# multimodallearning/DG-TTA

Measured on AMD Instinct MI355X. Metric: TTA-epochs/sec per GPU on 128^3 patch; Dice delta vs reference, higher is better.
Workload: dtype fp16

## Files before the change

dg_tta_amd/_lib.py:

```python
import ctypes as C
import os
from pathlib import Path

LIB_PATH = Path(__file__).resolve().parent / "libdgtta_hip.so"

_c_float_p = C.POINTER(C.c_float)
P, I, I64, F, SZ = C.c_void_p, C.c_int, C.c_int64, C.c_float, C.c_size_t

SIGNATURES = {
    "dgtta_version": (I, []),
    "dgtta_last_error": (C.c_char_p, []),
    "dgtta_reload_env": (I, []),
    "dgtta_mind3d_ws_bytes": (SZ, [I, I, I, I]),
    "dgtta_mind3d_fwd": (I, [P, P, F, I, C.POINTER(F), I, P, I, I, I, P, SZ, I, I, I, I, P]),
    "dgtta_gin_ws_bytes": (SZ, [I, I, I, I]),
    "dgtta_gin_chain_fwd": (I, [P, P, C.POINTER(I), C.POINTER(P), C.POINTER(P), P, P, SZ, I, I, I, I, P]),
    "dgtta_affine_warp3d_fwd": (I, [P, P, P, I, I, I, I, I, I, I, I, I, I, I, I, I, I, P, P]),
    "dgtta_affine_warp3d_bwd": (I, [P, P, P, I, I, I, I, I, I, I, I, I, I, I, I, I, P]),
    "dgtta_softdice_ws_bytes": (SZ, [I, I, I64]),
    "dgtta_softdice_fwd": (I, [P, P, P, P, P, SZ, I, I, I64, I, I, I, P]),
    "dgtta_softdice_bwd": (I, [P, P, P, P, P, F, P, I, I, I64, I, I, P]),
    "dgtta_softdice_bwd_t": (I, [P, P, P, P, P, F, P, I, I, I64, I, I, I, P]),
    "dgtta_softdice_probs_fwd": (I, [P, P, P, P, SZ, I, I, I64, I64, I64, I64, P]),
    "dgtta_softdice_probs_bwd": (I, [P, P, P, P, P, P, I, I, I64, I64, I64, I64, P]),
# ... 6 lines not shown
    "dgtta_conv3d_packed_bytes": (SZ, [I, I, I]),
    "dgtta_conv3d_pack_weights": (I, [P, P, I, I, I, I, I, P]),
    "dgtta_conv3d_stats_bytes": (SZ, [I, I, I, I, I]),
    "dgtta_conv3d_k3_fwd": (I, [P, I, P, P, P, I, P, I, I, I, I, I, I, I, I, I, I, I, P]),
    "dgtta_conv3d_k3_dgrad": (I, [P, I, P, P, I, I, I, I, I, I, I, I, I, I, I, I, I, P]),
    "dgtta_conv3d_wgrad_ws_bytes": (SZ, [I, I, I, I, I, I]),
    "dgtta_conv3d_wgrad_split_ws_bytes": (SZ, [I, I, I, I, I, I, I]),
    "dgtta_conv3d_k3_wgrad": (I, [P, I, P, I, P, P, P, SZ, I, I, I, I, I, I, I, I, I, I, P]),
    "dgtta_conv3d_k3_blocked_supported": (I, [I, I, I, I, I, I, I]),
    "dgtta_conv3d_k3_fwd_blocked": (I, [P, I64, P, P, P, I, P, I, I, I, I, I, I, I, I, I, P]),
    "dgtta_conv3d_k3_wgrad_blocked": (I, [P, I64, P, I, P, P, P, SZ, I, I, I, I, I, I, I, I, P]),
    "dgtta_instnorm_ws_bytes": (SZ, [I, I, I64]),
    "dgtta_instnorm_lrelu_fwd": (I, [P, I, P, P, P, P, P, I, P, SZ, I, I, I64, F, F, I, P]),
    "dgtta_instnorm_lrelu_bwd": (I, [P, I, P, I, P, P, P, P, I, P, P, P, SZ, I, I, I64, F, I, I, P]),
    "dgtta_conv3d_k3_dgrad_gstats": (I, [P, I, P, P, I, I, I, I, I, I, I, I, I, P, I, P, P, P, F, P, SZ, C.POINTER(I), I, I, P]),
    "dgtta_instnorm_lrelu_bwd_gstats": (I, [P, I, P, I, P, P, P, P, I, P, P, P, P, SZ, I, I, I64, F, I, I, P]),
    "dgtta_convT3d_fwd_ws_bytes": (SZ, [I, I, I]),
    "dgtta_convT3d_k2s2_fwd": (I, [P, I, P, P, P, I, P, SZ, I, I, I, I, I, I, I, I, P]),
    "dgtta_convT3d_bwd_ws_bytes": (SZ, [I, I, I, I, I, I]),
    "dgtta_convT3d_bwd_split_ws_bytes": (SZ, [I, I, I, I, I, I]),
    "dgtta_convT3d_k2s2_bwd": (I, [P, I, P, I, P, P, I, P, P, P, SZ, I, I, I, I, I, I, I, I, I, P]),
    "dgtta_seghead_fwd": (I, [P, I, P, P, P, I, P, I, I, I, I, I64, I, P]),
    "dgtta_seghead_bwd_ws_bytes": (SZ, [I, I, I, I64]),
    "dgtta_seghead_bwd": (I, [P, I, P, I, P, P, I, P, I, P, P, P, SZ, I, I, I64, I, I, P]),
    "dgtta_seghead_warp_supported": (I, [P, I, I, I, I, I, I, I]),
    "dgtta_seghead_warp_bwd_ws_bytes": (SZ, [I, I, I, I, I, I]),
    "dgtta_seghead_warp_fwd": (I, [P, P, P, P, I, P, P, I, I, I, I, I, I, I, P]),
    "dgtta_seghead_warp_bwd": (I, [P, P, P, P, P, P, I, P, P, P, P, SZ, I, I, I, I, I, I, I, I, P]),
    "dgtta_seghead_warp_bwd_g16": (I, [P, P, P, P, P, P, I, P, P, P, P, SZ, I, I, I, I, I, I, I, I, P]),
    "dgtta_ncdhw_to_ndhwc": (I, [P, P, I, I, I64, I, I, P]),
# ... 69 lines not shown
```

dg_tta_amd/csrc/common.h:

```cpp
#pragma once
#include <hip/hip_runtime.h>
#include <hip/hip_bf16.h>
#include <hip/hip_fp16.h>
#include <stdint.h>
#include <stdio.h>
#include <stdarg.h>

#include "../../include/dgtta.h"

#define WAVE 64

#include <atomic>

void dgtta_set_error(const char *fmt, ...);

struct DgttaSwitches {
  int conv_rows, conv_s2, dgrad_s2_allcls, wgrad_tr, wgrad_tr8, wgrad_s2_onepass, convt_wgrad_onepass;
  int convt_gemm, rows_order, in_nt, wgrad_upw, wgrad_xcd, in_gstats, softdice16, conv_ring, wgrad_ring, ha_mfma, wgrad_f32_split, feature_head_mfma, headwarp_mfma, wgrad_flat, wgrad_reduce_taps;
  int rows_abl, rows_var, ring_nt, ring_abl, wgrad_ring_lab, ha_abl, warp_abl, convt_gemm_abl;
  int ncu;
};
const DgttaSwitches &dgtta_switches();
#ifdef DGTTA_DIAG
#define DG_LAB(field) (dgtta_switches().field)
// ... 11 lines not shown
  (void)hipGetDevice(&dev);
  const unsigned long long bit = 1ull << (dev & 63);
  if (o.mask.load(std::memory_order_acquire) & bit) return hipSuccess;
  const hipError_t e = hipFuncSetAttribute(fn, hipFuncAttributeMaxDynamicSharedMemorySize, bytes);
  if (e == hipSuccess) o.mask.fetch_or(bit, std::memory_order_release);
  return e;
}

struct RowsGstCtx {
  const void *y;
  long long ldy;
  const float *mr, *gamma, *beta;
  float slope;
  double *out;
  int produced;
};

#define DG_REQUIRE(cond, code, ...)      \
  do {                                   \
    if (!(cond)) {                       \
      dgtta_set_error(__VA_ARGS__);      \
      return (code);                     \
    }                                    \
  } while (0)

#define DG_CHECK_LAUNCH(name)                                                     \
  do {                                                                            \
    hipError_t e__ = hipGetLastError();                                           \
    if (e__ != hipSuccess) {                                                      \
      dgtta_set_error("%s: launch failed: %s", name, hipGetErrorString(e__));     \
// ... 94 lines not shown
```

dg_tta_amd/csrc/conv_mfma.hip:

```cpp
#include "conv_common.h"
#include <stdlib.h>
#include <type_traits>

int conv3_rows_launch(const void *x, const View &xv, const void *w, const Taps &taps, const float *bias, void *y, const View &yv,
                      int B, int Cin, int Cout, int CinP, int CoutP, double *stats, int ntaps_src, int is_f16, hipStream_t st,
                      RowsGstCtx *gst);

int conv3_ring_launch(const void *x, const View &xv, const void *w, const Taps &taps, const float *bias, void *y, const View &yv,
                      int B, int Cin, int Cout, int CinP, int CoutP, double *stats, int64_t stats_cap_slots, int ntaps_src,
                      int is_f16, hipStream_t st, RowsGstCtx *gst, long long xkh = 0, bool dry = false);
int64_t conv3_mfma_max_tiles(int Do, int Ho, int Wo);

namespace {

template <typename T, int MBW, int MBH, int MBD, int S, int NB, int KSPC, int ABL = 0, int NW = 4, bool AC = false>
__global__ __launch_bounds__(NW * 64) void conv3_mfma_kernel(const T *__restrict__ x, View xv, const T *__restrict__ w,
                                                         ConvClasses cs, const float *__restrict__ bias,
                                                         T *__restrict__ y, View yv, int Cin, int Cout, int CinP,
                                                         int CoutP, int tilesW, int tilesH, int tilesD,
                                                         double *__restrict__ stats, int ntaps_src) {
  const int cls = blockIdx.z;
  x += cs.xoff[cls];
  if (!AC) y += cs.yoff[cls];
  const Taps &taps = cs.taps[cls];
  const int accumulate = cs.acc[cls];
  const int Di = xv.D, Hi = xv.H, Wi = xv.W, Do = yv.D, Ho = yv.H, Wo = yv.W;
  typedef ConvCfg<T, MBW, MBH, MBD, S, NB, KSPC> Cfg;
  typedef typename Cfg::G G;
  constexpr int EPV = Cfg::EPV, NG = Cfg::NG, CK = Cfg::CK, NC = Cfg::NC, NV = G::NV, MPW = G::MB / NW, NT = NW * 64;
  extern __shared__ __attribute__((aligned(16))) unsigned char smem[];
  uint4 *sA = reinterpret_cast<uint4 *>(smem);
  uint4 *sB = reinterpret_cast<uint4 *>(smem + Cfg::A_BYTES);

  const int tid = threadIdx.x, lane = tid & 63, wave = tid >> 6;
  const int r = lane & 31, h = lane >> 5;
// ... 158 lines not shown
            else mfma_step<T>(af, bf[j], acc[i][j]);
          }
        }
      }
    }
  }

  float st1[NB], st2[NB];
#pragma unroll
  for (int j = 0; j < NB; ++j) st1[j] = st2[j] = 0.f;
  if (AC) {
    const bool vec = Cout % 8 == 0 && (reinterpret_cast<uintptr_t>(y) & 15) == 0 && yv.sw % 8 == 0 && yv.sh % 8 == 0 &&
                     yv.sd % 8 == 0 && yv.sb % 8 == 0;
    __syncthreads();
    float *slab = reinterpret_cast<float *>(smem) + wave * (32 * 36);
#pragma unroll
    for (int i = 0; i < MPW; ++i) {
      const int mb = wave * MPW + i;
      const int mbd = mb / MBH, mbh = mb % MBH;
      const int co = n0 + r;
      uint4 olds[8][2];
      if constexpr (sizeof(T) == 2) {
        if (vec && accumulate) {
#pragma unroll
          for (int c8 = 0; c8 < 8; ++c8)
#pragma unroll
            for (int t = 0; t < 2; ++t) {
              const int m = t * 16 + (lane >> 2), cq = (lane & 3) * 8;
              const int od = od0 + mbd, oh = oh0 + mbh * G::RPM + m / MBW, ow = ow0 + m % MBW;
              olds[c8][t] = make_uint4(0u, 0u, 0u, 0u);
              if (n0 + cq < Cout && od < Do && oh < Ho && ow < Wo)
                olds[c8][t] = *reinterpret_cast<const uint4 *>(y + cs.yoff[c8] + b * yv.sb + od * yv.sd + oh * yv.sh + ow * yv.sw + n0 + cq);
            }
        }
      }
#pragma unroll
      for (int c8 = 0; c8 < 8; ++c8) {
        if (!vec) {
#pragma unroll
          for (int q = 0; q < 16; ++q) {
            const int m = (q & 3) + 8 * (q >> 2) + 4 * h;
            const int od = od0 + mbd, oh = oh0 + mbh * G::RPM + m / MBW, ow = ow0 + m % MBW;
            if (co < Cout && od < Do && oh < Ho && ow < Wo) {
              T *o = y + cs.yoff[c8] + b * yv.sb + od * yv.sd + oh * yv.sh + ow * yv.sw + co;
              float v = acc[i][c8][q];
              if (accumulate) v += ld_f<T>(o);
              st_f<T>(o, v);
            }
          }
          continue;
        }
#pragma unroll
// ... 14 lines not shown
                const unsigned wv[4] = {old.x, old.y, old.z, old.w};
#pragma unroll
                for (int e = 0; e < 4; ++e) {
                  float lo, hi;
                  unpack2_16<T>(wv[e], lo, hi);
                  v[2 * e] += lo;
                  v[2 * e + 1] += hi;
                }
              }
              uint4 pk;
              pk.x = pack2_16<T>(v[0], v[1]);
              pk.y = pack2_16<T>(v[2], v[3]);
              pk.z = pack2_16<T>(v[4], v[5]);
              pk.w = pack2_16<T>(v[6], v[7]);
              *o4 = pk;
            } else {
              float4 *o4 = reinterpret_cast<float4 *>(o);
              if (accumulate) {
                const float4 a0 = o4[0], a1 = o4[1];
                v[0] += a0.x; v[1] += a0.y; v[2] += a0.z; v[3] += a0.w;
                v[4] += a1.x; v[5] += a1.y; v[6] += a1.z; v[7] += a1.w;
              }
              o4[0] = make_float4(v[0], v[1], v[2], v[3]);
              o4[1] = make_float4(v[4], v[5], v[6], v[7]);
            }
          }
        }
      }
    }
    return;
  }
#pragma unroll
  for (int i = 0; i < MPW; ++i) {
    const int mb = wave * MPW + i;
    const int mbd = mb / MBH, mbh = mb % MBH;
#pragma unroll
    for (int j = 0; j < NB; ++j) {
      const int co = n0 + j * 32 + r;
      const float bv = (bias && co < Cout) ? bias[co] : 0.f;
#pragma unroll
      for (int q = 0; q < 16; ++q) {
        const int m = (q & 3) + 8 * (q >> 2) + 4 * h;
        const int od = od0 + mbd, oh = oh0 + mbh * G::RPM + m / MBW, ow = ow0 + m % MBW;
// ... 30 lines not shown
#pragma unroll
      for (int wv = 0; wv < NW; ++wv) {
        s += (double)red[(wv * NC + tid) * 2 + 0];
        ss += (double)red[(wv * NC + tid) * 2 + 1];
      }
      double *p = stats + 32 + (((int64_t)b * tiles_per_b + (tlin % tiles_per_b)) * Cout + n0 + tid) * 2;
      p[0] = s;
      p[1] = ss;
    }
    if (blockIdx.x == 0 && blockIdx.y == 0 && tid == 0) reinterpret_cast<long long *>(stats)[0] = tiles_per_b;
  }
}

template <typename T, int MBW, int MBH, int MBD>
int launch_conv_allcls(const void *x, const View &xv, const void *w, const ConvClasses &cs, void *y, const View &yv, int B,
                       int Cin, int Cout, int CinP, int CoutP, hipStream_t st) {
  typedef ConvCfg<T, MBW, MBH, MBD, 1, 1, 1> Cfg;
  typedef typename Cfg::G G;
  auto kern = conv3_mfma_kernel<T, MBW, MBH, MBD, 1, 1, 1, 0, 8, true>;
  static DynLdsOnce lds_once;
  DG_REQUIRE(ensure_dyn_lds(lds_once, reinterpret_cast<const void *>(kern), (int)Cfg::LDS_BYTES) == hipSuccess,
             DGTTA_ERR_LAUNCH, "conv3_mfma: cannot raise the dynamic LDS limit to %zu", (size_t)Cfg::LDS_BYTES);
  const int tW = cdiv(yv.W, G::TW), tH = cdiv(yv.H, G::TH), tD = cdiv(yv.D, G::TD);
  const int64_t tiles = (int64_t)tW * tH * tD * B;
  DG_REQUIRE(tiles < (1ll << 31), DGTTA_ERR_UNSUPPORTED, "conv3_mfma: too many tiles");
  dim3 grid((unsigned)tiles, (unsigned)cdiv(CoutP, Cfg::NC), 1u);
  hipLaunchKernelGGL(kern, grid, dim3(8 * 64), Cfg::LDS_BYTES, st, (const T *)x, xv, (const T *)w, cs, (const float *)nullptr,
                     (T *)y, yv, Cin, Cout, CinP, CoutP, tW, tH, tD, (double *)nullptr, 27);
  DG_CHECK_LAUNCH("conv3_mfma_kernel<all classes>");
  return DGTTA_OK;
}

template <typename T, int MBW, int MBH, int MBD, int S, int NB, int KSPC, int NW = 4>
int launch_conv(const void *x, const View &xv, const void *w, const ConvClasses &cs, const float *bias, void *y,
                const View &yv, int B, int Cin, int Cout, int CinP, int CoutP, double *stats, int ntaps_src,
                hipStream_t st) {
  typedef ConvCfg<T, MBW, MBH, MBD, S, NB, KSPC> Cfg;
  typedef typename Cfg::G G;
  auto kern = conv3_mfma_kernel<T, MBW, MBH, MBD, S, NB, KSPC, 0, NW>;
  static DynLdsOnce lds_once;
  DG_REQUIRE(ensure_dyn_lds(lds_once, reinterpret_cast<const void *>(kern), (int)Cfg::LDS_BYTES) == hipSuccess,
             DGTTA_ERR_LAUNCH, "conv3_mfma: cannot raise the dynamic LDS limit to %zu", (size_t)Cfg::LDS_BYTES);
  const int tW = cdiv(yv.W, G::TW), tH = cdiv(yv.H, G::TH), tD = cdiv(yv.D, G::TD);
  const int64_t tiles = (int64_t)tW * tH * tD * B;
  DG_REQUIRE(tiles < (1ll << 31), DGTTA_ERR_UNSUPPORTED, "conv3_mfma: too many tiles");
  dim3 grid((unsigned)tiles, (unsigned)cdiv(CoutP, Cfg::NC), (unsigned)cs.n);
  hipLaunchKernelGGL(kern, grid, dim3(NW * 64), Cfg::LDS_BYTES, st, (const T *)x, xv, (const T *)w, cs, bias, (T *)y, yv,
                     Cin, Cout, CinP, CoutP, tW, tH, tD, stats, ntaps_src);
  DG_CHECK_LAUNCH("conv3_mfma_kernel");
  return DGTTA_OK;
}

template <typename T>
int dispatch_conv_classes(const void *x, const View &xv, const void *w, const ConvClasses &cs, const float *bias, void *y,
                          const View &yv, int B, int Cin, int Cout, int CinP, int CoutP, int stride, hipStream_t st,
                          double *stats = nullptr, int ntaps_src = 27, RowsGstCtx *gst = nullptr, long long xkh = 0, bool dry = false) {
#define ARGS x, xv, w, cs, bias, y, yv, B, Cin, Cout, CinP, CoutP, stats, ntaps_src, st
  const long long vox = (long long)yv.D * yv.H * yv.W * B;
  if ((xkh || dry) && stride != 1) return DGTTA_ERR_UNSUPPORTED;
  if (stride == 0) {
    if (yv.W >= 32) return launch_conv<T, 32, 4, 4, 0, 1, 1, 8>(ARGS);
    if (yv.W >= 16) return launch_conv<T, 16, 4, 4, 0, 1, 1, 8>(ARGS);
    if (vox <= 4096) return launch_conv<T, 8, 2, 2, 0, 1, 1>(ARGS);
// ... 89 lines not shown
    if (i < nf) {
      int ci = (int)(i % CinP), co = (int)((i / CinP) % CoutN), tap = (int)(i / ((int64_t)CinP * CoutN));
      st_f<T>(imgF + conv_weight_image_index(co, ci, tap, CinP, 27, EPV),
              (ci < Cin && co < Cout) ? w[((int64_t)co * Cin + ci) * 27 + tap] : 0.f);
    }
    if (i < nb) {
      int co = (int)(i % CoutP), ci = (int)((i / CoutP) % CinN), tap = (int)(i / ((int64_t)CoutP * CinN));
      st_f<T>(imgB + conv_weight_image_index(ci, co, tap, CoutP, 27, EPV),
              (ci < Cin && co < Cout) ? w[((int64_t)co * Cin + ci) * 27 + tap] : 0.f);
    }
  }
}

}

int64_t conv3_mfma_max_tiles(int Do, int Ho, int Wo) {
  const int shapes[6][3] = {{4, 4, 32}, {4, 8, 16}, {2, 8, 8}, {8, 8, 8}, {4, 4, 16}, {4, 8, 8}};
  int64_t best = 0;
  for (auto &t : shapes) {
    int64_t n = (int64_t)cdiv(Do, t[0]) * cdiv(Ho, t[1]) * cdiv(Wo, t[2]);
    best = n > best ? n : best;
  }
  return best;
}

int conv3_s2_regs(const void *x, const View &xv, const void *wimg, const float *bias, void *y, const View &yv, int B, int Cin,
                  int Cout, int CinP, int CoutP, double *stats, int64_t cap_slots, int dtype, hipStream_t st);

int conv3_fwd_mfma(const void *x, int ldx, const void *w_kmajor, int mirror, const float *bias, void *y, int ldy, int B,
                   int Cin, int Cout, int CinP, int CoutP, int Di, int Hi, int Wi, int stride, int dtype,
// ... 12 lines not shown
    return dispatch_conv<float>(x, xv, w_kmajor, taps, bias, y, yv, B, Cin, Cout, CinP, CoutP, stride, 0, st, stats, 27, gst);
  }
  if (dtype == DGTTA_BF16) {
    if (!operand_ok<bf16_t>(x, xkh ? 2 * ldx : ldx, Cin, CinP)) return DGTTA_ERR_UNSUPPORTED;
    return dispatch_conv<bf16_t>(x, xv, w_kmajor, taps, bias, y, yv, B, Cin, Cout, CinP, CoutP, stride, 0, st, stats, 27, gst, xkh, dry);
  }
  if (dtype == DGTTA_F16) {
    if (!operand_ok<f16_t>(x, xkh ? 2 * ldx : ldx, Cin, CinP)) return DGTTA_ERR_UNSUPPORTED;
    return dispatch_conv<f16_t>(x, xv, w_kmajor, taps, bias, y, yv, B, Cin, Cout, CinP, CoutP, stride, 0, st, stats, 27, gst, xkh, dry);
  }
  return DGTTA_ERR_UNSUPPORTED;
}

template <typename T>
static int dgrad_s2(const void *dy, int lddy, const void *w_kmajor, void *dx, int lddx, int B, int Cin, int Cout, int CinP,
                    int CoutP, int Di, int Hi, int Wi, int accumulate, hipStream_t st) {
  if (!operand_ok<T>(dy, lddy, Cout, CoutP)) return DGTTA_ERR_UNSUPPORTED;
  const int Do = (Di - 1) / 2 + 1, Ho = (Hi - 1) / 2 + 1, Wo = (Wi - 1) / 2 + 1;
  const View xv = dense_view(B, Do, Ho, Wo, lddy);
  ConvClasses cs;
  cs.n = 8;
  cs.kseg = 0;
  View yv;
  for (int p = 0; p < 8; ++p) {
    const int pd = p >> 2, ph = (p >> 1) & 1, pw = p & 1;
    long long off;
    yv = parity_view(Di, Hi, Wi, lddx, pd, ph, pw, &off);
    yv.sb = (long long)Di * Hi * Wi * lddx;
    cs.xoff[p] = 0;
    cs.yoff[p] = off;
    cs.acc[p] = accumulate;
// ... 4 lines not shown
      for (int a = 0; a < 3; ++a) {
        if (par[a] == 0) {
          ok = ok && (k[a] == 1);
          real[a] = 1;
        } else {
          ok = ok && (k[a] >= 1);
          real[a] = (k[a] == 1) ? 2 : 0;
        }
      }
      cs.taps[p].wt[t] = ok ? (signed char)(real[0] * 9 + real[1] * 3 + real[2]) : (signed char)-1;
    }
  }
  {
    const int ac = dgtta_switches().dgrad_s2_allcls;
    if (ac != '0' && CinP % 8 == 0) {
      if (yv.W >= 32) return launch_conv_allcls<T, 32, 4, 2>(dy, xv, w_kmajor, cs, dx, yv, B, Cout, Cin, CoutP, CinP, st);
      if (yv.W >= 16) return launch_conv_allcls<T, 16, 2, 4>(dy, xv, w_kmajor, cs, dx, yv, B, Cout, Cin, CoutP, CinP, st);
      return launch_conv_allcls<T, 8, 2, 4>(dy, xv, w_kmajor, cs, dx, yv, B, Cout, Cin, CoutP, CinP, st);
    }
  }
  return dispatch_conv_classes<T>(dy, xv, w_kmajor, cs, nullptr, dx, yv, B, Cout, Cin, CoutP, CinP, 1, st);
}

int conv3_dgrad_s2_mfma(const void *dy, int lddy, const void *w_kmajor, void *dx, int lddx, int B, int Cin, int Cout,
                        int CinP, int CoutP, int Di, int Hi, int Wi, int accumulate, int dtype, hipStream_t st) {
  if (dtype == DGTTA_F32) return dgrad_s2<float>(dy, lddy, w_kmajor, dx, lddx, B, Cin, Cout, CinP, CoutP, Di, Hi, Wi, accumulate, st);
  if (dtype == DGTTA_BF16) return dgrad_s2<bf16_t>(dy, lddy, w_kmajor, dx, lddx, B, Cin, Cout, CinP, CoutP, Di, Hi, Wi, accumulate, st);
  if (dtype == DGTTA_F16) return dgrad_s2<f16_t>(dy, lddy, w_kmajor, dx, lddx, B, Cin, Cout, CinP, CoutP, Di, Hi, Wi, accumulate, st);
  return DGTTA_ERR_UNSUPPORTED;
}

static size_t n32(int c) { return (size_t)(c + 31) / 32 * 32; }
size_t convT_packed_bytes(int CinP, int CoutP, int dtype) {
  return (size_t)8 * (CinP * n32(CoutP) + CoutP * n32(CinP)) * (dtype == DGTTA_F32 ? 4 : 2);
}
size_t conv_image_bytes(int CinP, int CoutP, int dtype) {
  return (size_t)27 * (CinP * n32(CoutP) + CoutP * n32(CinP)) * (dtype == DGTTA_F32 ? 4 : 2);
}
size_t conv_imgB_offset_bytes(int CinP, int CoutP, int dtype) {
  return (size_t)27 * CinP * n32(CoutP) * (dtype == DGTTA_F32 ? 4 : 2);
}
int conv_pack_images(const float *w_t, void *img, int Cin, int Cout, int CinP, int CoutP, int dtype, hipStream_t st) {
  const int64_t n = (int64_t)27 * (CinP > CoutP ? CinP : CoutP) * n32(CinP > CoutP ? CinP : CoutP);
// ... 87 lines not shown
```

dg_tta_amd/csrc/unet_ref.hip:

```cpp
#include "common.h"

namespace {

template <typename T>
__global__ void pack_weights_kernel(const float *__restrict__ w, T *__restrict__ wf, T *__restrict__ wb, int Cin,
                                    int Cout, int CinP, int CoutP) {
  const int64_t nf = (int64_t)27 * CinP * CoutP;
  for (int64_t i = (int64_t)blockIdx.x * blockDim.x + threadIdx.x; i < nf; i += (int64_t)gridDim.x * blockDim.x) {
    {
      int co = (int)(i % CoutP), ci = (int)((i / CoutP) % CinP), tap = (int)(i / ((int64_t)CoutP * CinP));
      float v = (co < Cout && ci < Cin) ? w[((int64_t)co * Cin + ci) * 27 + tap] : 0.f;
      if (wf) st_f<T>(wf + i, v);
    }
    {
      int ci = (int)(i % CinP), co = (int)((i / CinP) % CoutP), tap = (int)(i / ((int64_t)CoutP * CinP));
      float v = (co < Cout && ci < Cin) ? w[((int64_t)co * Cin + ci) * 27 + (26 - tap)] : 0.f;
      if (wb) st_f<T>(wb + i, v);
    }
  }
}

template <typename T>
__global__ void conv3_fwd_ref_kernel(const T *__restrict__ x, int ldx, const T *__restrict__ wf,
                                     const float *__restrict__ bias, T *__restrict__ y, int ldy, int Cin, int Cout,
// ... 1105 lines not shown
      CALL;                                                                            \
    } else if ((dtype) == DGTTA_F16) {                                                 \
      typedef f16_t T;                                                                 \
      CALL;                                                                            \
    } else {                                                                           \
      dgtta_set_error("bad dtype %d", (int)(dtype));                                   \
      return DGTTA_ERR_BADARG;                                                         \
    }                                                                                  \
  } while (0)

int conv3_fwd_mfma(const void *x, int ldx, const void *w_kmajor, int mirror, const float *bias, void *y, int ldy, int B,
                   int Cin, int Cout, int CinP, int CoutP, int Di, int Hi, int Wi, int stride, int dtype,
                   hipStream_t st, double *stats, RowsGstCtx *gst = nullptr, long long xkh = 0, bool dry = false);
bool conv3_wgrad_blocked_ok(int B, int Cin, int Cout, int D, int H, int W, int dtype);
int64_t conv3_mfma_max_tiles(int Do, int Ho, int Wo);
int conv3_dgrad_s2_mfma(const void *dy, int lddy, const void *w_kmajor, void *dx, int lddx, int B, int Cin, int Cout,
                        int CinP, int CoutP, int Di, int Hi, int Wi, int accumulate, int dtype, hipStream_t st);
size_t convT_packed_bytes(int CinP, int CoutP, int dtype);
int convT_fwd_mfma(const void *x, int ldx, const float *w_t, const float *bias, void *out, int ldo, void *ws, int B, int Cin,
                   int Cout, int Di, int Hi, int Wi, int dtype, hipStream_t st);
int convT_dgrad_mfma(const void *dout, int lddo, const float *w_t, void *dx, int lddx, void *ws, int B, int Cin, int Cout,
                     int Di, int Hi, int Wi, int dtype, hipStream_t st);
int convT_wgrad_mfma(const void *x, int ldx, const void *dout, int lddo, float *dw_t, void *ws, size_t ws_bytes, int B,
                     int Cin, int Cout, int Di, int Hi, int Wi, int accumulate, int dtype, hipStream_t st, float *bias_part,
                     size_t bias_part_bytes, int *bias_units);
int convT_bias_finalize(const float *part, int units, int Cout, float *db, int accumulate, hipStream_t st);
int conv3_wgrad_mfma(const void *x, int ldx, const void *dy, int lddy, float *dw_t, float *db, void *ws, size_t ws_bytes,
                     int B, int Cin, int Cout, int Di, int Hi, int Wi, int stride, int accumulate, int dtype,
                     hipStream_t st, long long xkh = 0);

static size_t esize(int dtype) { return dtype == DGTTA_F32 ? 4 : 2; }
static const void *wb_of(const void *wpack, int CinP, int CoutP, int dtype) {
// ... 27 lines not shown
                                       w_t, (T *)wf, (T *)wb, Cin, Cout, CinP, CoutP));
  DG_CHECK_LAUNCH("pack_weights_kernel");
  if (CinP % (dtype == DGTTA_F32 ? 8 : 16) == 0 && CoutP % (dtype == DGTTA_F32 ? 8 : 16) == 0)
    return conv_pack_images(w_t, const_cast<void *>(img_of(wpack, CinP, CoutP, dtype)), Cin, Cout, CinP, CoutP, dtype,
                            (hipStream_t)stream);
  return DGTTA_OK;
}

static int out_dim(int i, int s) { return (i + 2 - 3) / s + 1; }

extern "C" size_t dgtta_conv3d_stats_bytes(int B, int Cout, int Do, int Ho, int Wo) {
  if (B <= 0 || Cout <= 0 || Do <= 0 || Ho <= 0 || Wo <= 0) return 0;
  int64_t nb = conv3_mfma_max_tiles(Do, Ho, Wo);
  const int64_t rb = reduce_blocks((int64_t)Do * Ho * Wo, B);
  if (rb > nb) nb = rb;
  return 256 + (size_t)B * nb * Cout * 2 * sizeof(double);
}

__global__ void set_header_kernel(long long *hdr, long long v) { hdr[0] = v; }

static int k3_fwd(const void *x, int ldx, long long x_block_stride, const void *wpack, const float *bias, void *y, int ldy,
                  void *stats, int B, int Cin, int Cout, int CinP, int CoutP, int Di, int Hi, int Wi, int stride, int dtype, int impl,
                  void *stream);

extern "C" int dgtta_conv3d_k3_fwd(const void *x, int ldx, const void *wpack, const float *bias, void *y, int ldy,
                                   void *stats, int B, int Cin, int Cout, int CinP, int CoutP, int Di, int Hi, int Wi,
                                   int stride, int dtype, int impl, void *stream) {
  return k3_fwd(x, ldx, 0, wpack, bias, y, ldy, stats, B, Cin, Cout, CinP, CoutP, Di, Hi, Wi, stride, dtype, impl, stream);
}

// ... 53 lines not shown
  DG_REQUIRE(dy && wpack && dx, DGTTA_ERR_BADARG, "conv3d_k3_dgrad: null pointer");
  const void *wb = wb_of(wpack, CinP, CoutP, dtype);
  DG_REQUIRE(B > 0 && Cin > 0 && Cout > 0 && CinP >= Cin && CoutP >= Cout && Di > 0 && Hi > 0 && Wi > 0,
             DGTTA_ERR_BADARG, "conv3d_k3_dgrad: bad dims");
  DG_REQUIRE(stride == 1 || stride == 2, DGTTA_ERR_UNSUPPORTED, "conv3d_k3_dgrad: stride %d", stride);
  DG_REQUIRE(lddx >= Cin && lddy >= Cout, DGTTA_ERR_BADARG, "conv3d_k3_dgrad: ld < C");
  hipStream_t st = (hipStream_t)stream;
  if (impl != 1 && stride == 1 && !accumulate) {
    int rc = conv3_fwd_mfma(dy, lddy, imgB_of(wpack, CinP, CoutP, dtype), 1, nullptr, dx, lddx, B, Cout, Cin, CoutP, CinP, Di,
                            Hi, Wi, 1, dtype, st, nullptr, gst);
    if (rc != DGTTA_ERR_UNSUPPORTED) return rc;
    DG_REQUIRE(impl == 0, DGTTA_ERR_UNSUPPORTED, "conv3d_k3_dgrad: shape not covered by the MFMA kernel");
  }
  if (impl != 1 && stride == 2 && !((Di | Hi | Wi) & 1)) {
    int rc = conv3_dgrad_s2_mfma(dy, lddy, imgB_of(wpack, CinP, CoutP, dtype), dx, lddx, B, Cin, Cout, CinP, CoutP, Di, Hi, Wi,
                                 accumulate, dtype, st);
    if (rc != DGTTA_ERR_UNSUPPORTED) return rc;
    DG_REQUIRE(impl == 0, DGTTA_ERR_UNSUPPORTED, "conv3d_k3_dgrad: shape not covered by the MFMA kernel");
  }
  const int Do = out_dim(Di, stride), Ho = out_dim(Hi, stride), Wo = out_dim(Wi, stride);
  const int64_t total = (int64_t)B * Di * Hi * Wi * Cin;
  DISPATCH_T(dtype, hipLaunchKernelGGL((conv3_dgrad_ref_kernel<T>), dim3(gs_blocks(total, 1 << 20)), dim3(256), 0, st,
                                       (const T *)dy, lddy, (const T *)wb, (T *)dx, lddx, Cin, Cout, CinP, CoutP, Di, Hi,
                                       Wi, Do, Ho, Wo, stride, accumulate, total));
  DG_CHECK_LAUNCH("conv3_dgrad_ref_kernel");
  return DGTTA_OK;
}

extern "C" int dgtta_conv3d_k3_dgrad(const void *dy, int lddy, const void *wpack, void *dx, int lddx, int B, int Cin,
                                     int Cout, int CinP, int CoutP, int Di, int Hi, int Wi, int stride, int accumulate,
                                     int dtype, int impl, void *stream) {
  return k3_dgrad(dy, lddy, wpack, dx, lddx, B, Cin, Cout, CinP, CoutP, Di, Hi, Wi, stride, accumulate, dtype, impl, stream, nullptr);
}


extern "C" int dgtta_conv3d_k3_dgrad_gstats(const void *dy, int lddy, const void *wpack, void *dx, int lddx, int B, int Cin,
                                            int Cout, int CinP, int CoutP, int Di, int Hi, int Wi, const void *y_prev,
                                            int ldy_prev, const float *mean_rstd_prev, const float *gamma_prev,
                                            const float *beta_prev, float slope, void *gstats, size_t gstats_bytes,
                                            int *h_produced, int dtype, int impl, void *stream) {
  DG_REQUIRE(y_prev && mean_rstd_prev && gamma_prev && beta_prev && gstats && h_produced, DGTTA_ERR_BADARG,
             "conv3d_k3_dgrad_gstats: null pointer");
  DG_REQUIRE(ldy_prev >= Cin, DGTTA_ERR_BADARG, "conv3d_k3_dgrad_gstats: ldy_prev < Cin");
  DG_REQUIRE(B > 0 && Cin > 0 && Di > 0 && Hi > 0 && Wi > 0 && gstats_bytes >= dgtta_conv3d_stats_bytes(B, Cin, Di, Hi, Wi),
             DGTTA_ERR_WORKSPACE, "conv3d_k3_dgrad_gstats: statistics buffer too small");
  RowsGstCtx ctx{y_prev, ldy_prev, mean_rstd_prev, gamma_prev, beta_prev, slope, (double *)gstats, 0};
  const bool fuse = dtype != DGTTA_F32 && impl != 1 && dgtta_switches().in_gstats != '0';
  const int rc = k3_dgrad(dy, lddy, wpack, dx, lddx, B, Cin, Cout, CinP, CoutP, Di, Hi, Wi, 1, 0, dtype, impl, stream,
                          fuse ? &ctx : nullptr);
  *h_produced = rc == DGTTA_OK ? ctx.produced : 0;
  return rc;
}

size_t conv3_wgrad_mfma_ws_bytes(int B, int Cin, int Cout, int D, int H, int W);
size_t conv3_wgrad_split_extra_bytes(int B, int Cin, int Cout, int D, int H, int W, int stride);

static size_t wgrad_bias_bytes(int B, int Cout, int Do, int Ho, int Wo) {
  return align_up((size_t)B * reduce_blocks((int64_t)Do * Ho * Wo, B) * Cout * 2 * sizeof(double), 256);
}

extern "C" size_t dgtta_conv3d_wgrad_ws_bytes(int B, int Cin, int Cout, int Do, int Ho, int Wo) {
  if (B <= 0 || Cin <= 0 || Cout <= 0 || Do <= 0 || Ho <= 0 || Wo <= 0) return 0;
  const int64_t nvox = (int64_t)B * Do * Ho * Wo;
// ... 485 lines not shown
```

dg_tta_amd/unet.py:

```python
import ctypes as C

import os

import torch
from torch import nn

from . import _lib
from ._lib import check, ptr, stream_of
from ._state import state_of
from .ops import F32, BF16, F16, _ws, dtype_code, is_cl3d

PLANS_3D_FULLRES = dict(features=(32, 64, 128, 256, 320), strides=(1, 2, 2, 2, 2),
                        n_conv_enc=(2, 2, 2, 2, 2), n_conv_dec=(2, 2, 2, 2),
                        in_channels=12, num_classes=105)
EPS, SLOPE = 1e-5, 1e-2


def _wgrad_on_side_stream():
    import os
    return os.environ.get("DGTTA_WGRAD_STREAM", "1") != "0"


def _pad(c, m):
    return (c + m - 1) // m * m
# ... 652 lines not shown
                                                     up["cin"], None, None, ptr(w_), nb, B, up["cin"], up["cout"],
                                                     ld0, lh0, lw0, ACC, dt, impl, st), "dgtta_convT3d_k2s2_bwd")
                    side.wait_event(ev)
                    gc.record_stream(side)
                    with torch.cuda.stream(side):
                        w2 = ws_for(nb, "ws_side")
                    check(lib.dgtta_convT3d_k2s2_bwd(up["x"], up["ldx"], ptr(gc), gc_ld, ptr(upm.weight), None,
                                                     up["cin"], ptr(dwu), ptr(dbu), ptr(w2), nb, B, up["cin"], up["cout"],
                                                     ld0, lh0, lw0, ACC, dt, impl, side.cuda_stream), "dgtta_convT3d_k2s2_bwd")
                gz_ptr, gz_ld = glow.data_ptr(), up["cin"]
                keep_alive = [glow, gc, gcat[sidx][0]]
            elif kind == "enc" and bidx == 0:
                prev_stage = sidx - 1
                dec_k = n_dec_stages - 1 - prev_stage
                gc, gptr, gld = gcat[dec_k]
                check(lib.dgtta_conv3d_k3_dgrad(ptr(dy), cout, ptr(wb), gptr, gld, B, cin, cout, rec["cinp"],
                                                rec["coutp"], di, hi, wi, s, 1, dt, impl, st), "dgtta_conv3d_k3_dgrad")
                gz_ptr, gz_ld = gptr, gld
                keep_alive = [gc]
            else:
                gin = torch.empty((B, di, hi, wi, cin), dtype=adt, device=dev)
                prev = saved[idx - 1]
                if s == 1 and dt != F32 and prev["cout"] == cin and prev["dout"] == (di, hi, wi):
                    pn = prev["mod"].norm
                    gbytes = lib.dgtta_conv3d_stats_bytes(B, cin, di, hi, wi)
                    gbuf_ = ws_for(gbytes, "gstats")
                    produced = C.c_int(0)
                    check(lib.dgtta_conv3d_k3_dgrad_gstats(ptr(dy), cout, ptr(wb), ptr(gin), cin, B, cin, cout, rec["cinp"],
                                                           rec["coutp"], di, hi, wi, ptr(prev["y"]), cin, ptr(prev["mr"]),
                                                           ptr(pn.weight), ptr(pn.bias), SLOPE, ptr(gbuf_), gbytes,
                                                           C.byref(produced), dt, impl, st), "dgtta_conv3d_k3_dgrad_gstats")
                    gstats = gbuf_ if produced.value else None
# ... 14 lines not shown
```

include/dgtta.h:

```cpp
#ifndef DGTTA_H
#define DGTTA_H

#include <stddef.h>
#include <stdint.h>

#ifdef __cplusplus
extern "C" {
#endif

#define DGTTA_OK 0
#define DGTTA_ERR_BADARG (-1)
#define DGTTA_ERR_UNSUPPORTED (-2)
#define DGTTA_ERR_WORKSPACE (-3)
#define DGTTA_ERR_LAUNCH (-4)

#define DGTTA_F32 0
#define DGTTA_BF16 1
#define DGTTA_F16 2

#define DGTTA_PAD_ZEROS 0
#define DGTTA_PAD_BORDER 1
#define DGTTA_INTERP_LINEAR 0
#define DGTTA_INTERP_NEAREST 1

// ... 71 lines not shown
                                  int dtype, void *stream);

size_t dgtta_instnorm_ws_bytes(int B, int C, int64_t V);
int dgtta_instnorm_lrelu_fwd(const void *y, int ldy, const void *stats, const float *gamma, const float *beta,
                             float *mean_rstd, void *z, int ldz, void *ws, size_t ws_bytes, int B, int C,
                             int64_t V, float eps, float slope, int dtype, void *stream);
int dgtta_instnorm_lrelu_bwd(const void *gz, int ldgz, const void *y, int ldy, const float *gamma,
                             const float *beta, const float *mean_rstd, void *dy, int lddy, float *dgamma,
                             float *dbeta, void *ws, size_t ws_bytes, int B, int C, int64_t V, float slope,
                             int accumulate, int dtype, void *stream);

int dgtta_conv3d_k3_dgrad_gstats(const void *dy, int lddy, const void *wpack, void *dx, int lddx, int B, int Cin, int Cout,
                                 int CinP, int CoutP, int Di, int Hi, int Wi, const void *y_prev, int ldy_prev,
                                 const float *mean_rstd_prev, const float *gamma_prev, const float *beta_prev, float slope,
                                 void *gstats, size_t gstats_bytes, int *h_produced, int dtype, int impl, void *stream);
int dgtta_instnorm_lrelu_bwd_gstats(const void *gz, int ldgz, const void *y, int ldy, const float *gamma, const float *beta,
                                    const float *mean_rstd, void *dy, int lddy, float *dgamma, float *dbeta,
                                    const void *gstats, void *ws, size_t ws_bytes, int B, int C, int64_t V, float slope,
                                    int accumulate, int dtype, void *stream);

size_t dgtta_convT3d_fwd_ws_bytes(int Cin, int Cout, int dtype);
int dgtta_convT3d_k2s2_fwd(const void *x, int ldx, const float *w_t, const float *bias, void *out, int ldo, void *ws,
                           size_t ws_bytes, int B, int Cin, int Cout, int Di, int Hi, int Wi, int dtype, int impl,
                           void *stream);
size_t dgtta_convT3d_bwd_ws_bytes(int B, int Cin, int Cout, int Di, int Hi, int Wi);
size_t dgtta_convT3d_bwd_split_ws_bytes(int B, int Cin, int Cout, int Di, int Hi, int Wi);
int dgtta_convT3d_k2s2_bwd(const void *x, int ldx, const void *dout, int lddo, const float *w_t, void *dx, int lddx,
                           float *dw_t, float *db, void *ws, size_t ws_bytes, int B, int Cin, int Cout, int Di,
                           int Hi, int Wi, int accumulate, int dtype, int impl, void *stream);

// ... 69 lines not shown
```

Before: 6.399.

## Fuse instance-norm backward gradient statistics into stride-2 all-class dgrad kernel

Extends the all-class stride-2 MFMA dgrad kernel with a template mode that, while writing dx, re-reads the previous layer's pre-norm activations and accumulates the per-channel LeakyReLU-masked gradient sums needed by the instance-norm backward. It adds a new C entry point and a Python call path for encoder stride-2 convs in fp16/bf16, so the later norm backward can skip its own full reduction pass over the gradient. In exchange the kernel does extra loads of y, more registers and LDS reductions, and a larger stats workspace.

New measurement: 6.446 (median of 5 runs). No clear change (+0.7%).

```diff
diff --git a/dg_tta_amd/_lib.py b/dg_tta_amd/_lib.py
--- a/dg_tta_amd/_lib.py
+++ b/dg_tta_amd/_lib.py
@@ -44,6 +44,7 @@
     "dgtta_instnorm_lrelu_fwd": (I, [P, I, P, P, P, P, P, I, P, SZ, I, I, I64, F, F, I, P]),
     "dgtta_instnorm_lrelu_bwd": (I, [P, I, P, I, P, P, P, P, I, P, P, P, SZ, I, I, I64, F, I, I, P]),
     "dgtta_conv3d_k3_dgrad_gstats": (I, [P, I, P, P, I, I, I, I, I, I, I, I, I, P, I, P, P, P, F, P, SZ, C.POINTER(I), I, I, P]),
+    "dgtta_conv3d_k3_dgrad_s2_gstats": (I, [P, I, P, P, I, I, I, I, I, I, I, I, I, I, P, I, P, P, P, F, P, SZ, C.POINTER(I), I, I, P]),
     "dgtta_instnorm_lrelu_bwd_gstats": (I, [P, I, P, I, P, P, P, P, I, P, P, P, P, SZ, I, I, I64, F, I, I, P]),
     "dgtta_convT3d_fwd_ws_bytes": (SZ, [I, I, I]),
     "dgtta_convT3d_k2s2_fwd": (I, [P, I, P, P, P, I, P, SZ, I, I, I, I, I, I, I, I, P]),
diff --git a/dg_tta_amd/csrc/common.h b/dg_tta_amd/csrc/common.h
--- a/dg_tta_amd/csrc/common.h
+++ b/dg_tta_amd/csrc/common.h
@@ -49,6 +49,7 @@
   float slope;
   double *out;
   int produced;
+  size_t bytes;
 };
 
 #define DG_REQUIRE(cond, code, ...)      \
diff --git a/dg_tta_amd/csrc/conv_mfma.hip b/dg_tta_amd/csrc/conv_mfma.hip
--- a/dg_tta_amd/csrc/conv_mfma.hip
+++ b/dg_tta_amd/csrc/conv_mfma.hip
@@ -13,12 +13,21 @@
 
 namespace {
 
-template <typename T, int MBW, int MBH, int MBD, int S, int NB, int KSPC, int ABL = 0, int NW = 4, bool AC = false>
+struct S2Gst {
+  const void *y;
+  long long sb, sd, sh, sw;
+  long long off[8];
+  const float *mr, *gamma, *beta;
+  float slope;
+};
+
+template <typename T, int MBW, int MBH, int MBD, int S, int NB, int KSPC, int ABL = 0, int NW = 4, bool AC = false,
+          bool GST = false>
 __global__ __launch_bounds__(NW * 64) void conv3_mfma_kernel(const T *__restrict__ x, View xv, const T *__restrict__ w,
                                                          ConvClasses cs, const float *__restrict__ bias,
                                                          T *__restrict__ y, View yv, int Cin, int Cout, int CinP,
                                                          int CoutP, int tilesW, int tilesH, int tilesD,
-                                                         double *__restrict__ stats, int ntaps_src) {
+                                                         double *__restrict__ stats, int ntaps_src, S2Gst gst) {
   const int cls = blockIdx.z;
   x += cs.xoff[cls];
   if (!AC) y += cs.yoff[cls];
@@ -207,12 +216,44 @@
                      yv.sd % 8 == 0 && yv.sb % 8 == 0;
     __syncthreads();
     float *slab = reinterpret_cast<float *>(smem) + wave * (32 * 36);
+    float *gcst = reinterpret_cast<float *>(smem) + NW * (32 * 36);
+    float gs1[8], gs2[8];
+    if constexpr (GST) {
+      static_assert(Cfg::LDS_BYTES >= (NW * 32 * 36 + 64) * sizeof(float), "GST constants do not fit behind the slabs");
+      if (tid < 32) {
+        const int c = n0 + tid;
+        const float mu = gst.mr[((long long)b * Cout + c) * 2], rs = gst.mr[((long long)b * Cout + c) * 2 + 1];
+        const float a = gst.gamma[c] * rs;
+        gcst[2 * tid] = a;
+        gcst[2 * tid + 1] = gst.beta[c] - mu * a;
+      }
+#pragma unroll
+      for (int e = 0; e < 8; ++e) gs1[e] = gs2[e] = 0.f;
+      __syncthreads();
+    }
 #pragma unroll
     for (int i = 0; i < MPW; ++i) {
       const int mb = wave * MPW + i;
       const int mbd = mb / MBH, mbh = mb % MBH;
       const int co = n0 + r;
       uint4 olds[8][2];
+      constexpr int GPF = 1;
+      uint4 gy[8][2];
+      auto load_gy = [&](int c8) {
+#pragma unroll
+        for (int t = 0; t < 2; ++t) {
+          const int m = t * 16 + (lane >> 2), cq = (lane & 3) * 8;
+          const int od = od0 + mbd, oh = oh0 + mbh * G::RPM + m / MBW, ow = ow0 + m % MBW;
+          gy[c8][t] = make_uint4(0u, 0u, 0u, 0u);
+          if (od < Do && oh < Ho && ow < Wo)
+            gy[c8][t] = *reinterpret_cast<const uint4 *>(reinterpret_cast<const T *>(gst.y) + gst.off[c8] + b * gst.sb +
+                                                         od * gst.sd + oh * gst.sh + ow * gst.sw + n0 + cq);
+        }
+      };
+      if constexpr (GST) {
+#pragma unroll
+        for (int c8 = 0; c8 < GPF; ++c8) load_gy(c8);
+      }
       if constexpr (sizeof(T) == 2) {
         if (vec && accumulate) {
 #pragma unroll
@@ -229,6 +270,9 @@
       }
 #pragma unroll
       for (int c8 = 0; c8 < 8; ++c8) {
+        if constexpr (GST) {
+          if (c8 + GPF < 8) load_gy(c8 + GPF);
+        }
         if (!vec) {
 #pragma unroll
           for (int q = 0; q < 16; ++q) {
@@ -273,6 +317,23 @@
               pk.z = pack2_16<T>(v[4], v[5]);
               pk.w = pack2_16<T>(v[6], v[7]);
               *o4 = pk;
+              if constexpr (GST) {
+                const uint4 yq = gy[c8][t];
+                const unsigned gw[4] = {pk.x, pk.y, pk.z, pk.w}, yw[4] = {yq.x, yq.y, yq.z, yq.w};
+#pragma unroll
+                for (int e = 0; e < 4; ++e) {
+                  float g0, g1, y0, y1;
+                  unpack2_16<T>(gw[e], g0, g1);
+                  unpack2_16<T>(yw[e], y0, y1);
+                  const float4 ab = *reinterpret_cast<const float4 *>(gcst + (cq + 2 * e) * 2);
+                  const float q0 = __builtin_fmaf(ab.x, y0, ab.y) > 0.f ? g0 : g0 * gst.slope;
+                  const float q1 = __builtin_fmaf(ab.z, y1, ab.w) > 0.f ? g1 : g1 * gst.slope;
+                  gs1[2 * e] += q0;
+                  gs1[2 * e + 1] += q1;
+                  gs2[2 * e] = __builtin_fmaf(q0, y0, gs2[2 * e]);
+                  gs2[2 * e + 1] = __builtin_fmaf(q1, y1, gs2[2 * e + 1]);
+                }
+              }
             } else {
               float4 *o4 = reinterpret_cast<float4 *>(o);
               if (accumulate) {
@@ -286,6 +347,38 @@
           }
         }
       }
+    }
+    if constexpr (GST) {
+#pragma unroll
+      for (int e = 0; e < 8; ++e)
+#pragma unroll
+        for (int m = 4; m < 64; m <<= 1) {
+          gs1[e] += __shfl_xor(gs1[e], m, 64);
+          gs2[e] += __shfl_xor(gs2[e], m, 64);
+        }
+      __syncthreads();
+      float *red = reinterpret_cast<float *>(smem);
+      if (lane < 4) {
+#pragma unroll
+        for (int e = 0; e < 8; ++e) {
+          red[(wave * 32 + lane * 8 + e) * 2 + 0] = gs1[e];
+          red[(wave * 32 + lane * 8 + e) * 2 + 1] = gs2[e];
+        }
+      }
+      __syncthreads();
+      const int tiles_per_b = tilesW * tilesH * tilesD;
+      if (tid < 32) {
+        double s = 0.0, ss = 0.0;
+#pragma unroll
+        for (int wv = 0; wv < NW; ++wv) {
+          s += (double)red[(wv * 32 + tid) * 2 + 0];
+          ss += (double)red[(wv * 32 + tid) * 2 + 1];
+        }
+        double *p = stats + 32 + (((int64_t)b * tiles_per_b + (tlin % tiles_per_b)) * Cout + n0 + tid) * 2;
+        p[0] = s;
+        p[1] = ss;
+      }
+      if (blockIdx.x == 0 && blockIdx.y == 0 && tid == 0) reinterpret_cast<long long *>(stats)[0] = tiles_per_b;
     }
     return;
   }
@@ -346,21 +439,31 @@
 
 template <typename T, int MBW, int MBH, int MBD>
 int launch_conv_allcls(const void *x, const View &xv, const void *w, const ConvClasses &cs, void *y, const View &yv, int B,
-                       int Cin, int Cout, int CinP, int CoutP, hipStream_t st) {
+                       int Cin, int Cout, int CinP, int CoutP, hipStream_t st, const S2Gst *gst = nullptr,
+                       double *gstats = nullptr) {
   typedef ConvCfg<T, MBW, MBH, MBD, 1, 1, 1> Cfg;
   typedef typename Cfg::G G;
+  static_assert(Cfg::LDS_BYTES >= 8 * 32 * 2 * sizeof(float), "GST reduction does not fit the LDS tiles");
   auto kern = conv3_mfma_kernel<T, MBW, MBH, MBD, 1, 1, 1, 0, 8, true>;
-  static DynLdsOnce lds_once;
-  DG_REQUIRE(ensure_dyn_lds(lds_once, reinterpret_cast<const void *>(kern), (int)Cfg::LDS_BYTES) == hipSuccess,
+  static DynLdsOnce lds_once, lds_once_gst;
+  DynLdsOnce *once = &lds_once;
+  if (gst) kern = conv3_mfma_kernel<T, MBW, MBH, MBD, 1, 1, 1, 0, 8, true, true>, once = &lds_once_gst;
+  DG_REQUIRE(ensure_dyn_lds(*once, reinterpret_cast<const void *>(kern), (int)Cfg::LDS_BYTES) == hipSuccess,
              DGTTA_ERR_LAUNCH, "conv3_mfma: cannot raise the dynamic LDS limit to %zu", (size_t)Cfg::LDS_BYTES);
   const int tW = cdiv(yv.W, G::TW), tH = cdiv(yv.H, G::TH), tD = cdiv(yv.D, G::TD);
   const int64_t tiles = (int64_t)tW * tH * tD * B;
   DG_REQUIRE(tiles < (1ll << 31), DGTTA_ERR_UNSUPPORTED, "conv3_mfma: too many tiles");
   dim3 grid((unsigned)tiles, (unsigned)cdiv(CoutP, Cfg::NC), 1u);
   hipLaunchKernelGGL(kern, grid, dim3(8 * 64), Cfg::LDS_BYTES, st, (const T *)x, xv, (const T *)w, cs, (const float *)nullptr,
-                     (T *)y, yv, Cin, Cout, CinP, CoutP, tW, tH, tD, (double *)nullptr, 27);
+                     (T *)y, yv, Cin, Cout, CinP, CoutP, tW, tH, tD, gstats, 27, gst ? *gst : S2Gst{});
   DG_CHECK_LAUNCH("conv3_mfma_kernel<all classes>");
   return DGTTA_OK;
+}
+
+template <int MBW, int MBH, int MBD>
+int64_t allcls_tiles(int Do, int Ho, int Wo) {
+  typedef typename ConvCfg<f16_t, MBW, MBH, MBD, 1, 1, 1>::G G;
+  return (int64_t)cdiv(Do, G::TD) * cdiv(Ho, G::TH) * cdiv(Wo, G::TW);
 }
 
 template <typename T, int MBW, int MBH, int MBD, int S, int NB, int KSPC, int NW = 4>
@@ -378,7 +481,7 @@
   DG_REQUIRE(tiles < (1ll << 31), DGTTA_ERR_UNSUPPORTED, "conv3_mfma: too many tiles");
   dim3 grid((unsigned)tiles, (unsigned)cdiv(CoutP, Cfg::NC), (unsigned)cs.n);
   hipLaunchKernelGGL(kern, grid, dim3(NW * 64), Cfg::LDS_BYTES, st, (const T *)x, xv, (const T *)w, cs, bias, (T *)y, yv,
-                     Cin, Cout, CinP, CoutP, tW, tH, tD, stats, ntaps_src);
+                     Cin, Cout, CinP, CoutP, tW, tH, tD, stats, ntaps_src, S2Gst{});
   DG_CHECK_LAUNCH("conv3_mfma_kernel");
   return DGTTA_OK;
 }
@@ -498,6 +601,13 @@
 
 }
 
+int64_t conv3_dgrad_s2_gst_tiles(int Di, int Hi, int Wi) {
+  const int Do = (Di - 1) / 2 + 1, Ho = (Hi - 1) / 2 + 1, Wo = (Wi - 1) / 2 + 1;
+  if (Wo >= 32) return allcls_tiles<32, 4, 2>(Do, Ho, Wo);
+  if (Wo >= 16) return allcls_tiles<16, 2, 4>(Do, Ho, Wo);
+  return allcls_tiles<8, 2, 4>(Do, Ho, Wo);
+}
+
 int64_t conv3_mfma_max_tiles(int Do, int Ho, int Wo) {
   const int shapes[6][3] = {{4, 4, 32}, {4, 8, 16}, {2, 8, 8}, {8, 8, 8}, {4, 4, 16}, {4, 8, 8}};
   int64_t best = 0;
@@ -540,7 +650,7 @@
 
 template <typename T>
 static int dgrad_s2(const void *dy, int lddy, const void *w_kmajor, void *dx, int lddx, int B, int Cin, int Cout, int CinP,
-                    int CoutP, int Di, int Hi, int Wi, int accumulate, hipStream_t st) {
+                    int CoutP, int Di, int Hi, int Wi, int accumulate, hipStream_t st, RowsGstCtx *gctx) {
   if (!operand_ok<T>(dy, lddy, Cout, CoutP)) return DGTTA_ERR_UNSUPPORTED;
   const int Do = (Di - 1) / 2 + 1, Ho = (Hi - 1) / 2 + 1, Wo = (Wi - 1) / 2 + 1;
   const View xv = dense_view(B, Do, Ho, Wo, lddy);
@@ -575,19 +685,40 @@
   {
     const int ac = dgtta_switches().dgrad_s2_allcls;
     if (ac != '0' && CinP % 8 == 0) {
-      if (yv.W >= 32) return launch_conv_allcls<T, 32, 4, 2>(dy, xv, w_kmajor, cs, dx, yv, B, Cout, Cin, CoutP, CinP, st);
-      if (yv.W >= 16) return launch_conv_allcls<T, 16, 2, 4>(dy, xv, w_kmajor, cs, dx, yv, B, Cout, Cin, CoutP, CinP, st);
-      return launch_conv_allcls<T, 8, 2, 4>(dy, xv, w_kmajor, cs, dx, yv, B, Cout, Cin, CoutP, CinP, st);
+      S2Gst g{};
+      const S2Gst *gp = nullptr;
+      double *gout = nullptr;
+      if (gctx && sizeof(T) == 2 && Cin % 32 == 0 && CinP == Cin && lddx % 8 == 0 && ((uintptr_t)dx & 15) == 0 &&
+          gctx->ldy % 8 == 0 && ((uintptr_t)gctx->y & 15) == 0 &&
+          gctx->bytes >= 256 + (size_t)B * conv3_dgrad_s2_gst_tiles(Di, Hi, Wi) * Cin * 2 * sizeof(double)) {
+        const long long ly = gctx->ldy;
+        g.y = gctx->y;
+        g.sb = (long long)Di * Hi * Wi * ly;
+        g.sd = 2ll * Hi * Wi * ly;
+        g.sh = 2ll * Wi * ly;
+        g.sw = 2 * ly;
+        for (int p = 0; p < 8; ++p) g.off[p] = (((long long)(p >> 2) * Hi + ((p >> 1) & 1)) * Wi + (p & 1)) * ly;
+        g.mr = gctx->mr;
+        g.gamma = gctx->gamma;
+        g.beta = gctx->beta;
+        g.slope = gctx->slope;
+        gp = &g;
+        gout = gctx->out;
+        gctx->produced = 1;
+      }
+      if (yv.W >= 32) return launch_conv_allcls<T, 32, 4, 2>(dy, xv, w_kmajor, cs, dx, yv, B, Cout, Cin, CoutP, CinP, st, gp, gout);
+      if (yv.W >= 16) return launch_conv_allcls<T, 16, 2, 4>(dy, xv, w_kmajor, cs, dx, yv, B, Cout, Cin, CoutP, CinP, st, gp, gout);
+      return launch_conv_allcls<T, 8, 2, 4>(dy, xv, w_kmajor, cs, dx, yv, B, Cout, Cin, CoutP, CinP, st, gp, gout);
     }
   }
   return dispatch_conv_classes<T>(dy, xv, w_kmajor, cs, nullptr, dx, yv, B, Cout, Cin, CoutP, CinP, 1, st);
 }
 
 int conv3_dgrad_s2_mfma(const void *dy, int lddy, const void *w_kmajor, void *dx, int lddx, int B, int Cin, int Cout,
-                        int CinP, int CoutP, int Di, int Hi, int Wi, int accumulate, int dtype, hipStream_t st) {
-  if (dtype == DGTTA_F32) return dgrad_s2<float>(dy, lddy, w_kmajor, dx, lddx, B, Cin, Cout, CinP, CoutP, Di, Hi, Wi, accumulate, st);
-  if (dtype == DGTTA_BF16) return dgrad_s2<bf16_t>(dy, lddy, w_kmajor, dx, lddx, B, Cin, Cout, CinP, CoutP, Di, Hi, Wi, accumulate, st);
-  if (dtype == DGTTA_F16) return dgrad_s2<f16_t>(dy, lddy, w_kmajor, dx, lddx, B, Cin, Cout, CinP, CoutP, Di, Hi, Wi, accumulate, st);
+                        int CinP, int CoutP, int Di, int Hi, int Wi, int accumulate, int dtype, hipStream_t st, RowsGstCtx *gctx) {
+  if (dtype == DGTTA_F32) return dgrad_s2<float>(dy, lddy, w_kmajor, dx, lddx, B, Cin, Cout, CinP, CoutP, Di, Hi, Wi, accumulate, st, nullptr);
+  if (dtype == DGTTA_BF16) return dgrad_s2<bf16_t>(dy, lddy, w_kmajor, dx, lddx, B, Cin, Cout, CinP, CoutP, Di, Hi, Wi, accumulate, st, gctx);
+  if (dtype == DGTTA_F16) return dgrad_s2<f16_t>(dy, lddy, w_kmajor, dx, lddx, B, Cin, Cout, CinP, CoutP, Di, Hi, Wi, accumulate, st, gctx);
   return DGTTA_ERR_UNSUPPORTED;
 }
 
diff --git a/dg_tta_amd/csrc/unet_ref.hip b/dg_tta_amd/csrc/unet_ref.hip
--- a/dg_tta_amd/csrc/unet_ref.hip
+++ b/dg_tta_amd/csrc/unet_ref.hip
@@ -1143,8 +1143,9 @@
                    hipStream_t st, double *stats, RowsGstCtx *gst = nullptr, long long xkh = 0, bool dry = false);
 bool conv3_wgrad_blocked_ok(int B, int Cin, int Cout, int D, int H, int W, int dtype);
 int64_t conv3_mfma_max_tiles(int Do, int Ho, int Wo);
+int64_t conv3_dgrad_s2_gst_tiles(int Di, int Hi, int Wi);
 int conv3_dgrad_s2_mfma(const void *dy, int lddy, const void *w_kmajor, void *dx, int lddx, int B, int Cin, int Cout,
-                        int CinP, int CoutP, int Di, int Hi, int Wi, int accumulate, int dtype, hipStream_t st);
+                        int CinP, int CoutP, int Di, int Hi, int Wi, int accumulate, int dtype, hipStream_t st, RowsGstCtx *gctx);
 size_t convT_packed_bytes(int CinP, int CoutP, int dtype);
 int convT_fwd_mfma(const void *x, int ldx, const float *w_t, const float *bias, void *out, int ldo, void *ws, int B, int Cin,
                    int Cout, int Di, int Hi, int Wi, int dtype, hipStream_t st);
@@ -1202,6 +1203,8 @@
   int64_t nb = conv3_mfma_max_tiles(Do, Ho, Wo);
   const int64_t rb = reduce_blocks((int64_t)Do * Ho * Wo, B);
   if (rb > nb) nb = rb;
+  const int64_t s2 = conv3_dgrad_s2_gst_tiles(Do, Ho, Wo);
+  if (s2 > nb) nb = s2;
   return 256 + (size_t)B * nb * Cout * 2 * sizeof(double);
 }
 
@@ -1285,7 +1288,7 @@
   }
   if (impl != 1 && stride == 2 && !((Di | Hi | Wi) & 1)) {
     int rc = conv3_dgrad_s2_mfma(dy, lddy, imgB_of(wpack, CinP, CoutP, dtype), dx, lddx, B, Cin, Cout, CinP, CoutP, Di, Hi, Wi,
-                                 accumulate, dtype, st);
+                                 accumulate, dtype, st, gst);
     if (rc != DGTTA_ERR_UNSUPPORTED) return rc;
     DG_REQUIRE(impl == 0, DGTTA_ERR_UNSUPPORTED, "conv3d_k3_dgrad: shape not covered by the MFMA kernel");
   }
@@ -1315,9 +1318,27 @@
   DG_REQUIRE(ldy_prev >= Cin, DGTTA_ERR_BADARG, "conv3d_k3_dgrad_gstats: ldy_prev < Cin");
   DG_REQUIRE(B > 0 && Cin > 0 && Di > 0 && Hi > 0 && Wi > 0 && gstats_bytes >= dgtta_conv3d_stats_bytes(B, Cin, Di, Hi, Wi),
              DGTTA_ERR_WORKSPACE, "conv3d_k3_dgrad_gstats: statistics buffer too small");
-  RowsGstCtx ctx{y_prev, ldy_prev, mean_rstd_prev, gamma_prev, beta_prev, slope, (double *)gstats, 0};
+  RowsGstCtx ctx{y_prev, ldy_prev, mean_rstd_prev, gamma_prev, beta_prev, slope, (double *)gstats, 0, gstats_bytes};
   const bool fuse = dtype != DGTTA_F32 && impl != 1 && dgtta_switches().in_gstats != '0';
   const int rc = k3_dgrad(dy, lddy, wpack, dx, lddx, B, Cin, Cout, CinP, CoutP, Di, Hi, Wi, 1, 0, dtype, impl, stream,
+                          fuse ? &ctx : nullptr);
+  *h_produced = rc == DGTTA_OK ? ctx.produced : 0;
+  return rc;
+}
+
+extern "C" int dgtta_conv3d_k3_dgrad_s2_gstats(const void *dy, int lddy, const void *wpack, void *dx, int lddx, int B, int Cin,
+                                               int Cout, int CinP, int CoutP, int Di, int Hi, int Wi, int accumulate,
+                                               const void *y_prev, int ldy_prev, const float *mean_rstd_prev,
+                                               const float *gamma_prev, const float *beta_prev, float slope, void *gstats,
+                                               size_t gstats_bytes, int *h_produced, int dtype, int impl, void *stream) {
+  DG_REQUIRE(y_prev && mean_rstd_prev && gamma_prev && beta_prev && gstats && h_produced, DGTTA_ERR_BADARG,
+             "conv3d_k3_dgrad_s2_gstats: null pointer");
+  DG_REQUIRE(ldy_prev >= Cin, DGTTA_ERR_BADARG, "conv3d_k3_dgrad_s2_gstats: ldy_prev < Cin");
+  DG_REQUIRE(B > 0 && Cin > 0 && Di > 0 && Hi > 0 && Wi > 0 && gstats_bytes >= dgtta_conv3d_stats_bytes(B, Cin, Di, Hi, Wi),
+             DGTTA_ERR_WORKSPACE, "conv3d_k3_dgrad_s2_gstats: statistics buffer too small");
+  RowsGstCtx ctx{y_prev, ldy_prev, mean_rstd_prev, gamma_prev, beta_prev, slope, (double *)gstats, 0, gstats_bytes};
+  const bool fuse = dtype != DGTTA_F32 && impl != 1 && dgtta_switches().in_gstats != '0';
+  const int rc = k3_dgrad(dy, lddy, wpack, dx, lddx, B, Cin, Cout, CinP, CoutP, Di, Hi, Wi, 2, accumulate, dtype, impl, stream,
                           fuse ? &ctx : nullptr);
   *h_produced = rc == DGTTA_OK ? ctx.produced : 0;
   return rc;
diff --git a/dg_tta_amd/unet.py b/dg_tta_amd/unet.py
--- a/dg_tta_amd/unet.py
+++ b/dg_tta_amd/unet.py
@@ -690,8 +690,20 @@
                 prev_stage = sidx - 1
                 dec_k = n_dec_stages - 1 - prev_stage
                 gc, gptr, gld = gcat[dec_k]
-                check(lib.dgtta_conv3d_k3_dgrad(ptr(dy), cout, ptr(wb), gptr, gld, B, cin, cout, rec["cinp"],
-                                                rec["coutp"], di, hi, wi, s, 1, dt, impl, st), "dgtta_conv3d_k3_dgrad")
+                prev = saved[idx - 1]
+                if s == 2 and dt != F32 and prev["cout"] == cin and prev["dout"] == (di, hi, wi):
+                    pn = prev["mod"].norm
+                    gbytes = lib.dgtta_conv3d_stats_bytes(B, cin, di, hi, wi)
+                    gbuf_ = ws_for(gbytes, "gstats")
+                    produced = C.c_int(0)
+                    check(lib.dgtta_conv3d_k3_dgrad_s2_gstats(ptr(dy), cout, ptr(wb), gptr, gld, B, cin, cout, rec["cinp"],
+                                                              rec["coutp"], di, hi, wi, 1, ptr(prev["y"]), cin, ptr(prev["mr"]),
+                                                              ptr(pn.weight), ptr(pn.bias), SLOPE, ptr(gbuf_), gbytes,
+                                                              C.byref(produced), dt, impl, st), "dgtta_conv3d_k3_dgrad_s2_gstats")
+                    gstats = gbuf_ if produced.value else None
+                else:
+                    check(lib.dgtta_conv3d_k3_dgrad(ptr(dy), cout, ptr(wb), gptr, gld, B, cin, cout, rec["cinp"],
+                                                    rec["coutp"], di, hi, wi, s, 1, dt, impl, st), "dgtta_conv3d_k3_dgrad")
                 gz_ptr, gz_ld = gptr, gld
                 keep_alive = [gc]
             else:
diff --git a/include/dgtta.h b/include/dgtta.h
--- a/include/dgtta.h
+++ b/include/dgtta.h
@@ -109,6 +109,11 @@
                                  int CinP, int CoutP, int Di, int Hi, int Wi, const void *y_prev, int ldy_prev,
                                  const float *mean_rstd_prev, const float *gamma_prev, const float *beta_prev, float slope,
                                  void *gstats, size_t gstats_bytes, int *h_produced, int dtype, int impl, void *stream);
+int dgtta_conv3d_k3_dgrad_s2_gstats(const void *dy, int lddy, const void *wpack, void *dx, int lddx, int B, int Cin, int Cout,
+                                    int CinP, int CoutP, int Di, int Hi, int Wi, int accumulate, const void *y_prev,
+                                    int ldy_prev, const float *mean_rstd_prev, const float *gamma_prev, const float *beta_prev,
+                                    float slope, void *gstats, size_t gstats_bytes, int *h_produced, int dtype, int impl,
+                                    void *stream);
 int dgtta_instnorm_lrelu_bwd_gstats(const void *gz, int ldgz, const void *y, int ldy, const float *gamma, const float *beta,
                                     const float *mean_rstd, void *dy, int lddy, float *dgamma, float *dbeta,
                                     const void *gstats, void *ws, size_t ws_bytes, int B, int C, int64_t V, float slope,
```
